# kuwt/edge_alignment

Hardware: AMD Instinct MI355X
Metric: edge-point residual+Jacobian evals/sec (higher is better)
Workload: dtype f64; 1 GPU; c2: single 640x480 frame pair, 50000 edge points, fp64, CauchyLoss(1); points_per_gpu=50000, dt_image=640x480, parallelism=independent frame pairs, one per GPU; single RCCL pose all-gather, tiles=196, points_per_thread=1, lds_bytes=0, point_order_tile_px=0

## Files before the change

### edge_alignment_amd/build.py

```python
import os
import shutil
import subprocess

_HERE = os.path.dirname(os.path.abspath(__file__))
SOURCES = [("csrc/ea_kernels.hip", ["-mllvm", "-amdgpu-sched-strategy=max-ilp"]), ("csrc/ea_kernels_var.hip", []),
           ("csrc/ea_preprocess.hip", []), ("csrc/ea_capi.hip", []), ("csrc/ea_frames.hip", []), ("csrc/ea_comm.hip", [])]
HEADERS = ["csrc/ea_types.h", "csrc/ea_lm.h", "csrc/ea_cov.h", "csrc/ea_prior.h", "csrc/ea_spin.h", "csrc/ea_hip_dev.h",
           "csrc/ea_launch.h", "csrc/ea_poses_map.h", "csrc/ea_wave_exchange.h", "csrc/ea_pair_log.h", "csrc/ea_starts_map.h", "csrc/ea_search_rank.h", "csrc/ea_select.h", "csrc/ea_frame_ws.h", "csrc/ea_capi_internal.h", "../include/ea_hip.h"]
LIB = os.path.join(_HERE, "lib", "libea_hip.so")
FLAGS = ["--offload-arch=gfx950", "-O3", "-std=c++17", "-fno-slp-vectorize", "-fPIC", "-mllvm", "-amdgpu-kernarg-preload-count=16",
         "-Wall", "-Wno-unused-function"]


def _hipcc():
    for cand in (os.environ.get("HIPCC"), "/opt/rocm/bin/hipcc", shutil.which("hipcc")):
        if cand and os.path.exists(cand):
            return cand
    raise RuntimeError("hipcc not found")


def build_library(force=False, verbose=False, out=None, defines=()):
    lib = out or LIB
    srcs = [os.path.join(_HERE, s) for s, _ in SOURCES]
    deps = srcs + [os.path.join(_HERE, h) for h in HEADERS]
    if (not force and os.path.exists(lib)
            and all(os.path.getmtime(lib) >= os.path.getmtime(d) for d in deps)):
        return lib
    obj_dir = os.path.join(os.path.dirname(lib), "obj" + ("_" + os.path.basename(lib) if out else ""))
    os.makedirs(obj_dir, exist_ok=True)
    cc = _hipcc()
    procs, objs = [], []
    for (src, extra), path in zip(SOURCES, srcs):
        obj = os.path.join(obj_dir, os.path.basename(src) + ".o")
        cmd = [cc] + FLAGS + list(extra) + ["-D" + d for d in defines] + ["-c", "-o", obj, path]
        if verbose:
            print(" ".join(cmd))
        procs.append((cmd, subprocess.Popen(cmd, cwd=_HERE)))
        objs.append(obj)
    for cmd, pr in procs:
        if pr.wait() != 0:
            raise subprocess.CalledProcessError(pr.returncode, cmd)
    link = [cc, "--offload-arch=gfx950", "-fPIC", "-shared", "-o", lib] + objs + ["-ldl"]
    if verbose:
        print(" ".join(link))
    subprocess.check_call(link, cwd=_HERE)
    return lib


if __name__ == "__main__":
    print(build_library(force=True, verbose=True))
```

### edge_alignment_amd/csrc/ea_kernels.hip

```cpp

#include <hip/hip_runtime.h>

#include <cstddef>
#include <type_traits>

#if defined(EA_STAMPS) && defined(__HIP_DEVICE_COMPILE__)
namespace ea {
extern __device__ unsigned long long *g_lm_stamp_buf;
extern __device__ int g_lm_probe_row;
}
#define EA_LM_PROBE(k)                                                                              \
  do {                                                                                              \
    if (g_lm_stamp_buf && blockIdx.x == 0) {                                                        \
      unsigned long long t_;                                                                        \
      __builtin_amdgcn_sched_barrier(0);                                                            \
      asm volatile("s_memtime %0\n\ts_waitcnt lgkmcnt(0)" : "=s"(t_)::"memory");                    \
      __builtin_amdgcn_sched_barrier(0);                                                            \
      g_lm_stamp_buf[64 * 8 + g_lm_probe_row * 8 + (k)] = t_;                                       \
    }                                                                                               \
  } while (0)
#endif
#include "ea_launch.h"
#include "ea_poses_map.h"
#include "ea_starts_map.h"
#include "ea_lm.h"
#include "ea_pair_log.h"
#include "ea_prior.h"
#include "ea_select.h"
#include "ea_types.h"
#include "ea_wave_exchange.h"

namespace ea {

#ifdef EA_STAMPS
__device__ unsigned long long *g_stamp_buf = nullptr;
#ifndef EA_STAMPS_EVAL
#define EA_STAMP(slot) do {} while (0)
#else
#define EA_STAMP(slot)                                                                              \
  do {                                                                                              \
    if (g_stamp_buf && threadIdx.x == 0) {                                                          \
      unsigned long long t_;                                                                        \
      __builtin_amdgcn_sched_barrier(0);                                                            \
      asm volatile("s_memtime %0\n\ts_waitcnt lgkmcnt(0)" : "=s"(t_)::"memory");                    \
      __builtin_amdgcn_sched_barrier(0);                                                            \
      g_stamp_buf[((size_t)blockIdx.y * gridDim.x + blockIdx.x) * 8 + (slot)] = t_;                 \
    }                                                                                               \
  } while (0)
#endif
__device__ unsigned long long *g_lm_stamp_buf = nullptr;
__device__ int g_lm_probe_row = 0;
#define EA_LM_STAMP(slot, eval)                                                                     \
  do {                                                                                              \
    if (g_lm_stamp_buf && threadIdx.x == 0 && blockIdx.x == 0) {                                    \
      unsigned long long t_;                                                                        \
      __builtin_amdgcn_sched_barrier(0);                                                            \
      asm volatile("s_memtime %0\n\ts_waitcnt lgkmcnt(0)" : "=s"(t_)::"memory");                    \
      __builtin_amdgcn_sched_barrier(0);                                                            \
      g_lm_stamp_buf[((eval) & 63) * 8 + (slot)] = t_;                                              \
    }                                                                                               \
  } while (0)
#define EA_LM_CLOCK(var)                                                                            \
  unsigned long long var = 0;                                                                       \
  do {                                                                                              \
    __builtin_amdgcn_sched_barrier(0);                                                              \
    asm volatile("s_memtime %0\n\ts_waitcnt lgkmcnt(0)" : "=s"(var)::"memory");                    \
    __builtin_amdgcn_sched_barrier(0);                                                              \
  } while (0)
#define EA_LM_STAMP_PUT(slot, eval, var)                                                            \
  do {                                                                                              \
    if (g_lm_stamp_buf && threadIdx.x == 0 && blockIdx.x == 0) g_lm_stamp_buf[((eval) & 63) * 8 + (slot)] = var; \
  } while (0)
#else
#define EA_STAMP(slot) do {} while (0)
#define EA_LM_STAMP(slot, eval) do {} while (0)
#define EA_LM_CLOCK(var) do {} while (0)
#define EA_LM_STAMP_PUT(slot, eval, var) do {} while (0)
#endif


template <typename T> __device__ __forceinline__ T t_rcp(T x);
template <> __device__ __forceinline__ float t_rcp<float>(float x) { return __builtin_amdgcn_rcpf(x); }
template <> __device__ __forceinline__ double t_rcp<double>(double x) {
  double r = __builtin_amdgcn_rcp(x);
  double e = __builtin_fma(-x, r, 1.0);
  r = __builtin_fma(r, e, r);
  e = __builtin_fma(-x, r, 1.0);
  return __builtin_fma(r, e, r);
}

template <typename T> __device__ __forceinline__ T t_log(T x);
template <> __device__ __forceinline__ float t_log<float>(float x) { return __builtin_amdgcn_logf(x) * 0.6931471805599453f; }

__device__ __forceinline__ double s_const(double c) { asm("" : "+s"(c)); return c; }
__device__ __forceinline__ float s_const(float c) { return c; }

struct LogOps {
  static __device__ __forceinline__ double frexp_mant(double x) { return __builtin_amdgcn_frexp_mant(x); }
  static __device__ __forceinline__ int frexp_exp(double x) { return __builtin_amdgcn_frexp_exp(x); }
  static __device__ __forceinline__ double ldexp(double x, int e) { return __builtin_amdgcn_ldexp(x, e); }
  static __device__ __forceinline__ double rcp(double x) { return __builtin_amdgcn_rcp(x); }
  static __device__ __forceinline__ double sconst(double c) { return s_const(c); }
};
template <> __device__ __forceinline__ double t_log<double>(double x) { return pl_log<LogOps>(x); }

template <typename T> __device__ __forceinline__ T t_sqrt(T x);
template <> __device__ __forceinline__ float t_sqrt<float>(float x) { return __builtin_amdgcn_sqrtf(x); }
template <> __device__ __forceinline__ double t_sqrt<double>(double x) { return sqrt(x); }

template <typename T> __device__ __forceinline__ T t_fma(T a, T b, T c) { return __builtin_fma(a, b, c); }
template <> __device__ __forceinline__ float t_fma<float>(float a, float b, float c) { return __builtin_fmaf(a, b, c); }

template <typename T>
__device__ __forceinline__ void cr_weights(T x, T w[4], T d[4]) {
  const T x2 = x * x;
  const T c15 = s_const(T(1.5));
  w[0] = x * t_fma<T>(x, t_fma<T>(T(-0.5), x, T(1)), T(-0.5));
  w[1] = t_fma<T>(x2, t_fma<T>(c15, x, T(-2.5)), T(1));
  w[2] = x * t_fma<T>(x, t_fma<T>(-c15, x, T(2)), T(0.5));
  w[3] = x2 * t_fma<T>(T(0.5), x, T(-0.5));
  const T c45 = s_const(T(4.5));
  d[0] = t_fma<T>(x, t_fma<T>(-c15, x, T(2)), T(-0.5));
  d[1] = x * t_fma<T>(c45, x, T(-5));
  d[2] = t_fma<T>(x, t_fma<T>(-c45, x, T(4)), T(0.5));
  d[3] = x * t_fma<T>(c15, x, T(-1));
}

template <typename T> struct Uni;
template <> struct Uni<double> {
  static __device__ __forceinline__ const double *R(const PoseState &ps) { return ps.R; }
  static __device__ __forceinline__ const double *t(const PoseState &ps) { return ps.t; }
  static __device__ __forceinline__ const double *G(const PoseState &ps) { return ps.G; }
  static __device__ __forceinline__ double fx(const ProblemDesc &pd) { return pd.fx; }
  static __device__ __forceinline__ double fy(const ProblemDesc &pd) { return pd.fy; }
  static __device__ __forceinline__ double cx(const ProblemDesc &pd) { return pd.cx; }
  static __device__ __forceinline__ double cy(const ProblemDesc &pd) { return pd.cy; }
  static __device__ __forceinline__ double loss_a(const ProblemDesc &pd) { return pd.loss_a; }
  static __device__ __forceinline__ double loss_inv_b(const ProblemDesc &pd) { return pd.loss_inv_b; }
  static __device__ __forceinline__ double z_guard(const ProblemDesc &pd) { return pd.z_guard; }
  static __device__ __forceinline__ double z_eps(const ProblemDesc &pd) { return pd.z_eps; }
  static __device__ __forceinline__ const double *dist(const ProblemDesc &pd) { return pd.dist; }
  static __device__ __forceinline__ const double *A(const ProblemDesc &pd) { return pd.A; }
  static __device__ __forceinline__ const double *d(const ProblemDesc &pd) { return pd.d; }
  static __device__ __forceinline__ const double *Ai(const ProblemDesc &pd) { return pd.Ai; }
  static __device__ __forceinline__ const double *di(const ProblemDesc &pd) { return pd.di; }
};
template <> struct Uni<float> {
  static __device__ __forceinline__ const float *R(const PoseState &ps) { return ps.Rf; }
  static __device__ __forceinline__ const float *t(const PoseState &ps) { return ps.tf; }
  static __device__ __forceinline__ const float *G(const PoseState &ps) { return ps.Gf; }
  static __device__ __forceinline__ float fx(const ProblemDesc &pd) { return pd.fxf; }
  static __device__ __forceinline__ float fy(const ProblemDesc &pd) { return pd.fyf; }
  static __device__ __forceinline__ float cx(const ProblemDesc &pd) { return pd.cxf; }
  static __device__ __forceinline__ float cy(const ProblemDesc &pd) { return pd.cyf; }
  static __device__ __forceinline__ float loss_a(const ProblemDesc &pd) { return pd.loss_af; }
  static __device__ __forceinline__ float loss_inv_b(const ProblemDesc &pd) { return pd.loss_inv_bf; }
  static __device__ __forceinline__ float z_guard(const ProblemDesc &pd) { return pd.z_guardf; }
  static __device__ __forceinline__ float z_eps(const ProblemDesc &pd) { return pd.z_epsf; }
  static __device__ __forceinline__ const float *dist(const ProblemDesc &pd) { return pd.distf; }
  static __device__ __forceinline__ const float *A(const ProblemDesc &pd) { return pd.Af; }
  static __device__ __forceinline__ const float *d(const ProblemDesc &pd) { return pd.df; }
  static __device__ __forceinline__ const float *Ai(const ProblemDesc &pd) { return pd.Aif; }
  static __device__ __forceinline__ const float *di(const ProblemDesc &pd) { return pd.dif; }
};

template <typename T>
struct PoseLite {
  T R[9], t[3];
  int unit_q;
  const PoseState *full;
};
template <typename T> struct PoseAcc {
  static __device__ __forceinline__ const T *R(const PoseState &ps) { return Uni<T>::R(ps); }
  static __device__ __forceinline__ const T *t(const PoseState &ps) { return Uni<T>::t(ps); }
// ... 1236 lines not shown
        v[u] = *reinterpret_cast<const D2 *>(partials + (size_t)min(base + j + u * G, last) * kAccSlots + 2 * id);
    };
    auto add_round = [&](int base, const D2(&v)[U]) {
#pragma unroll
      for (int u = 0; u < U; ++u) {
        const bool in = base + j + u * G <= last;
        s[u].x += in ? v[u].x : 0.0;
        s[u].y += in ? v[u].y : 0.0;
      }
    };
    D2 v0[U], v1[U];
    load_round(tile_begin, v0);
    if (tile_begin + U * G <= last) {
      load_round(tile_begin + U * G, v1);
      add_round(tile_begin, v0);
      add_round(tile_begin + U * G, v1);
      for (int base = tile_begin + 2 * U * G; base <= last; base += U * G) {
        load_round(base, v0);
        add_round(base, v0);
      }
    } else {
      add_round(tile_begin, v0);
    }
  }
#pragma unroll
  for (int w = 1; w < U; w *= 2)
#pragma unroll
    for (int u = 0; u + w < U; u += 2 * w) s[u] += s[u + w];
  *reinterpret_cast<D2 *>(s_part + j * kAccSlots + 2 * id) = s[0];
  __syncthreads();
  if constexpr (F == 1) {
    if (tid < kAccSlots) {
      double tot = 0.0;
#pragma unroll
      for (int k = 0; k < G; ++k) tot += s_part[k * kAccSlots + tid];
      out[tid] = tot;
    }
  } else {
    double *s_fin = s_part + G * kAccSlots;
    if (tid < kAccSlots * F) {
      const int slot = tid & 31, f = tid >> 5;
      double tot = 0.0;
#pragma unroll
      for (int k = 0; k < 16; ++k) tot += s_part[(16 * f + k) * kAccSlots + slot];
      s_fin[f * kAccSlots + slot] = tot;
    }
    __syncthreads();
    if (tid < kAccSlots) {
      double tot = 0.0;
#pragma unroll
      for (int f = 0; f < F; ++f) tot += s_fin[f * kAccSlots + tid];
      out[tid] = tot;
    }
  }
}

__global__ __launch_bounds__(kFoldThreads) void ea_reduce_kernel(const GroupDesc *__restrict__ groups,
                                                                  const double *__restrict__ partials,
                                                                  EvalOut *__restrict__ out) {
  __shared__ __align__(16) double s_part[reduce_tiles_lds<kFoldThreads>()];
  const GroupDesc gd = groups[blockIdx.x];
  reduce_tiles<kFoldThreads, 4>(partials, gd.tile_begin, gd.tile_end, s_part, out[blockIdx.x].acc);
}

__device__ __forceinline__ void signal_done(unsigned int *counter, unsigned int n, int *host_flag, int seq) {
  __threadfence_system();
  const unsigned int prev = __hip_atomic_fetch_add(counter, 1u, __ATOMIC_ACQ_REL, __HIP_MEMORY_SCOPE_AGENT);
  if (prev == n - 1u) {
    __hip_atomic_store(counter, 0u, __ATOMIC_RELAXED, __HIP_MEMORY_SCOPE_AGENT);
    __threadfence_system();
    __hip_atomic_store(host_flag, seq, __ATOMIC_RELEASE, __HIP_MEMORY_SCOPE_SYSTEM);
  }
}

__global__ __launch_bounds__(kFoldThreads) void ea_reduce_done_kernel(const GroupDesc *__restrict__ groups,
                                                                       const double *__restrict__ partials,
                                                                       EvalOut *__restrict__ out, unsigned int *__restrict__ counter,
                                                                       int *__restrict__ host_flag, int seq) {
  __shared__ __align__(16) double s_part[reduce_tiles_lds<kFoldThreads>()];
  const GroupDesc gd = groups[blockIdx.x];
  reduce_tiles<kFoldThreads, 4>(partials, gd.tile_begin, gd.tile_end, s_part, out[blockIdx.x].acc);
  if (threadIdx.x == 0) signal_done(counter, gridDim.x, host_flag, seq);
}

__global__ __launch_bounds__(kLmThreads) void ea_reduce256_kernel(const GroupDesc *__restrict__ groups,
                                                                  const double *__restrict__ partials,
                                                                  EvalOut *__restrict__ out) {
  __shared__ __align__(16) double s_part[reduce_tiles_lds<kLmThreads>()];
  const GroupDesc gd = groups[blockIdx.x];
  reduce_tiles<kLmThreads, 4>(partials, gd.tile_begin, gd.tile_end, s_part, out[blockIdx.x].acc);
}

template <typename T, int PPT, int NT, bool BUF, bool IMG32 = false>
__global__ __launch_bounds__(NT) void ea_eval_fold_kernel(
    const void *__restrict__ x0, const void *__restrict__ y0, const void *__restrict__ z0, int n0,
    int shape, int chunks_per_xcd,
    const ProblemDesc *__restrict__ probs, const PoseState *__restrict__ poses,
    double *__restrict__ partials, int lds_texels,
    const GroupDesc *__restrict__ groups, const double *__restrict__ prev_rows, EvalOut *__restrict__ prev_out) {
  if (blockIdx.x == gridDim.x - 1) {
    __shared__ __align__(16) double s_part[reduce_tiles_lds<NT>()];
    const GroupDesc gd = groups[blockIdx.y];
    reduce_tiles<NT, 4>(prev_rows, gd.tile_begin, gd.tile_end, s_part, prev_out[blockIdx.y].acc);
    return;
  }
  eval_fused_body<T, PPT, 0, NT, false, BUF, IMG32>(x0, y0, z0, n0, shape, chunks_per_xcd, probs, poses, partials, lds_texels);
}

template <int NT>
__device__ __forceinline__ void poses_fold_one(const PosesFold &f, int r) {
  __shared__ __align__(16) double s_part[reduce_tiles_lds<NT>()];
  int pose, problem;
  poses_rider(r, f.count, &pose, &problem);
  const GroupDesc gd = f.groups[problem];
  const int base = pose * f.rows_per_pose;
  reduce_tiles<NT, 4>(f.rows, base + gd.tile_begin, base + gd.tile_end, s_part, f.out[r].acc);
  if (threadIdx.x == 0) signal_done(f.counter, (unsigned)f.n, f.host_flag, f.seq);
}

template <typename T, int PPT, int MODE, int NT, bool VAR, bool BUF, bool IMG32 = false>
__global__ __launch_bounds__(NT) void ea_eval_poses_kernel(
    const void *__restrict__ x0, const void *__restrict__ y0, const void *__restrict__ z0, int n0,
    int shape, int g, int rows,
    const ProblemDesc *__restrict__ probs, const PoseState *__restrict__ poses,
    double *__restrict__ partials, PosesFold fold) {
  static_assert((MODE == 0 || MODE == kModeExchange) && !VAR, "plain functor, stencil rows from L2");
  constexpr bool XCHG = MODE == kModeExchange;
  extern __shared__ __align__(16) unsigned char smem[];
  double *s_red = reinterpret_cast<double *>(smem);
  int *s_box = reinterpret_cast<int *>(smem + kRedBytes);
  const PosesWork w = poses_work(blockIdx.x, shape, rows, g, fold.n);
  if (w.kind != 2) {
    if (w.kind == 1) poses_fold_one<NT>(fold, w.rider);
    return;
  }
  const PosesChunk pc = poses_chunk(w, shape, rows, reinterpret_cast<const PosesRow *>(probs) - rows);
  const int tid = threadIdx.x;
  EA_ITEM_HEAD(false, NT * PPT, pc.chunk, pc.term, pc.slot, false, return);
  const double sum = fused_chunk<T, PPT, 0, NT, false, BUF, IMG32, PoseLite<T>, XCHG>(pd, ps, X, Y, Z, count, s_red, s_box, (T *)nullptr, 0,
                                                                                       tid < kAccSlots ? tid : -1);
  store_row_sum<XCHG>(partials, pc.out_row, sum);
}

template <int NT>
__global__ __launch_bounds__(NT) void ea_poses_fold_kernel(PosesFold fold) {
  poses_fold_one<NT>(fold, blockIdx.x);
}

template <typename T> using CPtr = const T __attribute__((address_space(4))) *;
constexpr int kLanesWaves = 4, kLanesSub = 512 / kLanesWaves, kLanesVals = 29;

template <typename IT> struct LanesStage {
  double cx_, cy_, cz_, iz, fu, fv;
  bool valid;
  Row4<IT> row[4];
};
template <typename IT> __device__ __forceinline__ Row4<double> lanes_widen(const Row4<IT> &r) {
  Row4<double> o;
  o.p0 = (double)r.p0; o.p1 = (double)r.p1; o.p2 = (double)r.p2; o.p3 = (double)r.p3;
  return o;
}
template <bool BUF, bool IMG32>
__device__ __forceinline__ void lanes_stage(const ProblemDesc &pd, const PoseLite<double> &ps, double x, double y, double z,
                                            bool inb, LanesStage<typename ImgOf<double, IMG32>::type> &st, int &n_bad) {
  typedef double T;
  typedef typename ImgOf<T, IMG32>::type IT;
  const int pitch = pd.pitch;
  const void *img_base = IMG32 ? pd.dt32 : pd.dt;
  Proj<T> pr;
  project_point<T>(pd, ps, x, y, z, pr);
  st.valid = inb && pr.state == 1;
  n_bad += (inb && pr.state == 2) ? 1 : 0;
  if (__any(!st.valid)) {
    asm volatile("" ::: "memory");
    if (!st.valid) { pr.iu = 0; pr.iv = 0; pr.fu = T(0); pr.fv = T(0); }
  }
  st.cx_ = pr.cx_; st.cy_ = pr.cy_; st.cz_ = pr.cz_; st.iz = pr.iz; st.fu = pr.fu; st.fv = pr.fv;
  if constexpr (BUF) {
    const __amdgpu_buffer_rsrc_t rimg =
        make_raw_buffer(img_base, (unsigned)pitch * (unsigned)(pd.H + 2 * kImagePad) * (unsigned)sizeof(IT));
    const int voff = ((pr.iv + (kImagePad - 1)) * pitch + (pr.iu + (kImagePad - 1))) * (int)sizeof(IT);
#pragma unroll
    for (int l = 0; l < 4; ++l) st.row[l] = buf_load_row4<IT>(rimg, voff, l * pitch * (int)sizeof(IT));
  } else {
    const GPtr<IT> gimg = (GPtr<IT>)(static_cast<const IT *>(img_base) + (size_t)kImagePad * (size_t)pitch + kImagePad);
    const GPtr<IT> base = gimg + ((ptrdiff_t)(pr.iv - 1) * pitch + (pr.iu - 1));
#pragma unroll
    for (int l = 0; l < 4; ++l) st.row[l] = load_row4<IT>(base + (ptrdiff_t)l * pitch);
  }
}
struct LanesLogRun { double P, L; int E; };
template <bool IMG32, bool UNIT>
__device__ __forceinline__ void lanes_sums(int k, const ProblemDesc &pd, const PoseLite<double> &ps_, double x, double y, double z,
                                           const LanesStage<typename ImgOf<double, IMG32>::type> &st, bool pair,
                                           double (&acc)[28], double &cost, double &held, LanesLogRun &run,
                                           const double (*s_pose)[64]) {
  typedef double T;
  PoseLite<T> ps = ps_;
  if constexpr (UNIT) ps.unit_q = 1;
  const T loss_a = Uni<T>::loss_a(pd);
  Proj<T> pr;
  pr.cx_ = st.cx_; pr.cy_ = st.cy_; pr.cz_ = st.cz_; pr.iz = st.iz; pr.fu = st.fu; pr.fv = st.fv;
  if constexpr (UNIT) {
    asm volatile("" ::: "memory");
    ps.t[0] = s_pose[10][threadIdx.x & 63]; ps.t[1] = s_pose[11][threadIdx.x & 63];
  }
  pr.bx = st.cx_ + ps.t[0]; pr.by = st.cy_ + ps.t[1];
  pr.fxz = Uni<T>::fx(pd) * st.iz; pr.fyz = Uni<T>::fy(pd) * st.iz;
  if (__any(!st.valid)) {
    asm volatile("" ::: "memory");
    if (!st.valid) {
      pr.iz = T(1);
      pr.bx = T(0); pr.by = T(0);
      pr.fxz = T(0); pr.fyz = T(0);
    }
  }
  T f, Fu, Fv;
  bicubic<T>(pr.fu, pr.fv, [&](int l) { return lanes_widen(st.row[l]); }, f, Fu, Fv);
  T J[6];
  jacobian_row<T>(pd, ps, pr, x, y, z, Fu, Fv, J);
  T rho, w;
  if (UNIT && pair) {
    const T xs = (f * f) * Uni<T>::loss_inv_b(pd);
    rho = xs + T(1);
    w = t_rcp<T>(rho);
    if (__any(!st.valid)) {
      asm volatile("" ::: "memory");
      if (!st.valid) { w = T(0); rho = T(1); }
    }
    T p = run.P * rho;
    const bool high = pl_run_high<LogOps>(p);
    if (__any(high)) {
      asm volatile("" ::: "memory");
      if (high) p = pl_run_renorm<LogOps>(run.P, run.L, run.E, rho);
    }
    pl_run_take(run.P, run.L, rho, p);
  } else {
    loss_point<T, 2, false>(pair, pd.loss_kind, loss_a, Uni<T>::loss_inv_b(pd), f * f, st.valid, T(1), rho, w);
  }
  const T wr = w * f;
  int s = 0;
#pragma unroll
  for (int a = 0; a < 6; ++a) {
    const T wJa = w * J[a];
#pragma unroll
    for (int b = a; b < 6; ++b) { acc[s] = t_fma<T>(wJa, J[b], acc[s]); ++s; }
    acc[kAccJtr + a] = t_fma<T>(J[a], wr, acc[kAccJtr + a]);
  }
  if (!(UNIT && pair)) cost_point<T, 2>(k, pair, loss_a, rho, cost, held);
}

template <bool BUF, bool IMG32, bool UNIT>
__device__ __forceinline__ void lanes_run(const ProblemDesc &pd, const PoseLite<double> &ps_, CPtr<double> px, CPtr<double> py,
                                          CPtr<double> pz, int n_sub, bool pair, double (&acc)[28], int &n_bad,
                                          const double (*s_pose)[64]) {
  typedef double T;
  typedef typename ImgOf<T, IMG32>::type IT;
  if (n_sub <= 0) return;
  const int lane = threadIdx.x & 63;
  n_sub = __builtin_amdgcn_readfirstlane(n_sub);
  const int last = n_sub - 1;
  LanesLogRun run = {T(1), T(0), 0};
  T X[2], Y[2], Z[2], NX[2], NY[2], NZ[2];
  {
    const int i1 = min(1, last), i2 = min(2, last), i3 = min(3, last);
    X[0] = px[0]; X[1] = px[i1]; Y[0] = py[0]; Y[1] = py[i1]; Z[0] = pz[0]; Z[1] = pz[i1];
    NX[0] = px[i2]; NX[1] = px[i3]; NY[0] = py[i2]; NY[1] = py[i3]; NZ[0] = pz[i2]; NZ[1] = pz[i3];
  }
#pragma nounroll
  for (int i = 0; i < n_sub; i += 2) {
    const int i4 = min(i + 4, last), i5 = min(i + 5, last);
    const T FX[2] = {px[i4], px[i5]}, FY[2] = {py[i4], py[i5]}, FZ[2] = {pz[i4], pz[i5]};
    T held = T(1), cost = T(0);
    LanesStage<IT> A, B;
    PoseLite<T> ps = ps_;
    if constexpr (UNIT) {
      asm volatile("" ::: "memory");
#pragma unroll
      for (int k = 0; k < 9; ++k) ps.R[k] = s_pose[k][lane];
      ps.t[2] = s_pose[9][lane]; ps.t[0] = s_pose[10][lane]; ps.t[1] = s_pose[11][lane];
    }
    lanes_stage<BUF, IMG32>(pd, ps, X[0], Y[0], Z[0], true, A, n_bad);
    if constexpr (UNIT) lanes_stage<BUF, IMG32>(pd, ps, X[1], Y[1], Z[1], i + 1 < n_sub, B, n_bad);
    lanes_sums<IMG32, UNIT>(0, pd, ps, X[0], Y[0], Z[0], A, pair, acc, cost, held, run, s_pose);
    if constexpr (!UNIT) lanes_stage<BUF, IMG32>(pd, ps, X[1], Y[1], Z[1], i + 1 < n_sub, B, n_bad);
    lanes_sums<IMG32, UNIT>(1, pd, ps, X[1], Y[1], Z[1], B, pair, acc, cost, held, run, s_pose);
    if (!(UNIT && pair)) acc[kAccCost] += cost;
#pragma unroll
    for (int k = 0; k < 2; ++k) { X[k] = NX[k]; Y[k] = NY[k]; Z[k] = NZ[k]; NX[k] = FX[k]; NY[k] = FY[k]; NZ[k] = FZ[k]; }
  }
  if (UNIT && pair) acc[kAccCost] = (T(0.5) * (Uni<T>::loss_a(pd) * Uni<T>::loss_a(pd))) * pl_run_log<LogOps>(run.P, run.L, run.E);
}

__device__ __forceinline__ bool lanes_ticket(unsigned int *counter, unsigned int target, volatile int *s_word) {
  asm volatile("s_waitcnt vmcnt(0)" ::: "memory");
  __syncthreads();
  if (threadIdx.x == 0) {
    __builtin_amdgcn_fence(__ATOMIC_RELEASE, "agent");
    asm volatile("s_waitcnt vmcnt(0)" ::: "memory");
    const unsigned int prev = __hip_atomic_fetch_add(counter, 1u, __ATOMIC_RELAXED, __HIP_MEMORY_SCOPE_AGENT);
    const int last = prev + 1u == target;
    if (last) {
      __builtin_amdgcn_fence(__ATOMIC_ACQUIRE, "agent");
      asm volatile("s_waitcnt vmcnt(0)" ::: "memory");
    }
    *s_word = last;
  }
  __syncthreads();
  return *s_word != 0;
}
constexpr int kLanesFoldSlots = (kLanesVals + kLanesWaves - 1) / kLanesWaves;
__device__ __forceinline__ void lanes_fold_blocks(const double *src, size_t stride, int n, int wave, int lane, double (&v)[kLanesFoldSlots]) {
#pragma unroll
  for (int j = 0; j < kLanesFoldSlots; ++j) v[j] = 0.0;
  const double *p = src + lane;
  int r = 0;
  for (; r + 4 <= n; r += 4) {
    double x[4][kLanesFoldSlots];
#pragma unroll
    for (int u = 0; u < 4; ++u)
#pragma unroll
      for (int j = 0; j < kLanesFoldSlots; ++j) {
        const int slot = wave + kLanesWaves * j;
        x[u][j] = slot < kLanesVals ? p[(size_t)(r + u) * stride + (size_t)slot * kPosesLanes] : 0.0;
      }
#pragma unroll
    for (int u = 0; u < 4; ++u)
#pragma unroll
      for (int j = 0; j < kLanesFoldSlots; ++j) v[j] += x[u][j];
  }
  for (; r < n; ++r) {
    double x[kLanesFoldSlots];
#pragma unroll
    for (int j = 0; j < kLanesFoldSlots; ++j) {
      const int slot = wave + kLanesWaves * j;
      x[j] = slot < kLanesVals ? p[(size_t)r * stride + (size_t)slot * kPosesLanes] : 0.0;
    }
#pragma unroll
    for (int j = 0; j < kLanesFoldSlots; ++j) v[j] += x[j];
  }
}
__device__ __forceinline__ void lanes_tickets(const PosesTickets &tk, const double *rows_base, int rows, int group, int problem,
                                              int row0, int nrows, int chunk, int pose0, int live, int groups, double *s_lds) {
  const int lane = threadIdx.x & 63, wave = __builtin_amdgcn_readfirstlane(threadIdx.x >> 6);
  volatile int *s_word = reinterpret_cast<volatile int *>(s_lds);
  const int count = tk.count, run = poses_lanes_run(chunk), slot1 = poses_lanes_run_slot(row0, problem, run);
  if (!lanes_ticket(tk.counters + poses_lanes_counter1(group, slot1, rows, count), (unsigned)poses_lanes_run_rows(nrows, run), s_word)) return;
  double v[kLanesFoldSlots];
  lanes_fold_blocks(rows_base + poses_lanes_row_off(group, row0 + run * kPosesRun, rows), (size_t)kPosesLanesBlock,
                    poses_lanes_run_rows(nrows, run), wave, lane, v);
  double *part = tk.partials + poses_lanes_partial_off(group, slot1, rows, count);
#pragma unroll
  for (int j = 0; j < kLanesFoldSlots; ++j) {
    const int slot = wave + kLanesWaves * j;
    if (slot < kLanesVals) part[(size_t)slot * kPosesLanes + lane] = v[j];
  }
  if (!lanes_ticket(tk.counters + poses_lanes_counter2(groups, group, problem, rows, count), (unsigned)poses_lanes_runs(nrows), s_word)) return;
  lanes_fold_blocks(tk.partials + poses_lanes_partial_off(group, poses_lanes_run_slot(row0, problem, 0), rows, count),
                    (size_t)kPosesLanesBlock, poses_lanes_runs(nrows), wave, lane, v);
  __syncthreads();
  static_assert(kLanesFoldSlots * kLanesWaves == kAccSlots, "the wavefronts' slots cover a result exactly");
#pragma unroll
  for (int j = 0; j < kLanesFoldSlots; ++j) {
    const int slot = wave + kLanesWaves * j;
    s_lds[slot * 65 + lane] = slot < kLanesVals ? v[j] : 0.0;
  }
  __syncthreads();
  {
    const int s = threadIdx.x & (kAccSlots - 1), p0 = threadIdx.x / kAccSlots;
#pragma unroll
    for (int it = 0; it < kPosesLanes / (64 * kLanesWaves / kAccSlots); ++it) {
      const int p = p0 + it * (64 * kLanesWaves / kAccSlots);
      if (p < live) tk.out[(size_t)(pose0 + p) * (size_t)count + (size_t)problem].acc[s] = s_lds[s * 65 + p];
    }
  }
  __threadfence_system();
  __syncthreads();
  if (threadIdx.x == 0) {
    __threadfence_system();
    __hip_atomic_store(tk.flags + poses_lanes_flag(tk.group0 + group, problem, count), tk.seq, __ATOMIC_RELEASE, __HIP_MEMORY_SCOPE_SYSTEM);
  }
}

template <bool BUF, bool IMG32>
__global__ __launch_bounds__(64 * kLanesWaves) __attribute__((amdgpu_waves_per_eu(2, 2))) void ea_eval_poses_lanes_kernel(
    int shape, int g, int rows, const ProblemDesc *__restrict__ probs, const PoseState *__restrict__ poses,
    double *rows_out, PosesTickets tk) {
  typedef double T;
  __shared__ __align__(16) double s_sum[kLanesWaves / 2][kLanesVals][64];
  __shared__ __align__(16) double s_pose[kLanesWaves][12][64];
  static_assert(sizeof(s_sum) >= sizeof(double) * kAccSlots * 65, "the fold's transposition fits the sums' array");
  const PosesLanesWork w = poses_lanes_work(blockIdx.x, shape, rows, g, 0);
  if (w.kind != 2) return;
  const PosesLanesChunk pc = poses_lanes_chunk(w.row, shape, reinterpret_cast<const PosesRow *>(probs) - rows);
  const ProblemDesc pd = probs[pc.term];
  const long long start = (long long)pc.chunk * (kLanesWaves * kLanesSub);
  const int count = (int)max(0ll, min((long long)(kLanesWaves * kLanesSub), (long long)pd.n - start));
  const int lane = threadIdx.x & 63, wave = __builtin_amdgcn_readfirstlane(threadIdx.x >> 6);
  const PoseState *psp = poses + ((size_t)(w.pose0 + min(lane, w.live - 1)) * (size_t)pc.count + (size_t)pc.term);
  PoseLite<T> ps;
  int active;
  load_pose_lite<T>(psp, ps, active);
  const bool on = lane < w.live && active != 0;

  T v[kLanesVals];
#pragma unroll
  for (int i = 0; i < kLanesVals; ++i) v[i] = T(0);
  if (__any(on)) {
    const int first = wave * kLanesSub, n_sub = max(0, min(kLanesSub, count - first));
    const CPtr<T> px = (CPtr<T>)(static_cast<const T *>(pd.x) + start + first);
    const CPtr<T> py = (CPtr<T>)(static_cast<const T *>(pd.y) + start + first);
    const CPtr<T> pz = (CPtr<T>)(static_cast<const T *>(pd.z) + start + first);
    const bool pair = pd.loss_kind == 1;
    T acc[28];
#pragma unroll
    for (int i = 0; i < 28; ++i) acc[i] = T(0);
    int n_bad = 0;
#pragma unroll
    for (int k = 0; k < 9; ++k) s_pose[wave][k][lane] = ps.R[k];
    s_pose[wave][9][lane] = ps.t[2]; s_pose[wave][10][lane] = ps.t[0]; s_pose[wave][11][lane] = ps.t[1];
    if (__all(ps.unit_q != 0)) lanes_run<BUF, IMG32, true>(pd, ps, px, py, pz, n_sub, pair, acc, n_bad, s_pose[wave]);
    else lanes_run<BUF, IMG32, false>(pd, ps, px, py, pz, n_sub, pair, acc, n_bad, s_pose[wave]);

#pragma unroll
    for (int i = 0; i < 28; ++i) v[i] = acc[i];
    v[28] = (T)n_bad;
#pragma unroll
    for (int s = 1; s < kLanesWaves; s <<= 1) {
      const int role = wave & (2 * s - 1), buf = wave / (2 * s);
      if (role == s) {
#pragma unroll
        for (int i = 0; i < kLanesVals; ++i) s_sum[buf][i][lane] = v[i];
      }
      __syncthreads();
      if (role == 0) {
#pragma unroll
        for (int i = 0; i < kLanesVals; ++i) v[i] += s_sum[buf][i][lane];
      }
      if (2 * s < kLanesWaves) __syncthreads();
    }
  }
  const int group = w.pose0 / kPosesLanes;
  if (wave == 0) {
    double *o = rows_out + poses_lanes_row_off(group, w.row, rows) + lane;
#pragma unroll
    for (int i = 0; i < kLanesVals; ++i) o[(size_t)i * kPosesLanes] = on ? v[i] : 0.0;
  }
  if (!tk.on) return;
  lanes_tickets(tk, rows_out, rows, group, pc.term, w.row - pc.chunk, pd.tile_end - pd.tile_begin, pc.chunk, w.pose0, w.live,
                poses_lanes_groups(g), &s_sum[0][0][0]);
}


template <typename T>
__device__ __forceinline__ void cr_weights_value(T x, T w[4]) {
  const T x2 = x * x;
  const T c15 = s_const(T(1.5));
  w[0] = x * t_fma<T>(x, t_fma<T>(T(-0.5), x, T(1)), T(-0.5));
  w[1] = t_fma<T>(x2, t_fma<T>(c15, x, T(-2.5)), T(1));
  w[2] = x * t_fma<T>(x, t_fma<T>(-c15, x, T(2)), T(0.5));
  w[3] = x2 * t_fma<T>(T(0.5), x, T(-0.5));
}
template <typename T, typename RowFn>
__device__ __forceinline__ T bicubic_value(T fu, T fv, RowFn row) {
  T wu[4], wv[4];
  cr_weights_value<T>(fu, wu);
  cr_weights_value<T>(fv, wv);
  T f = T(0);
#pragma unroll
  for (int l = 0; l < 4; ++l) {
    const Row4<T> r = row(l);
    const T rs = t_fma<T>(wu[3], r.p3, t_fma<T>(wu[2], r.p2, t_fma<T>(wu[1], r.p1, wu[0] * r.p0)));
    f = t_fma<T>(wv[l], rs, f);
  }
  return f;
}

template <int CTRL> __device__ __forceinline__ int lane_xchg(int x) { return __builtin_amdgcn_update_dpp(0, x, CTRL, 0xF, 0xF, true); }
template <int W>
__device__ __forceinline__ void swap_rows_b32(unsigned &a, unsigned &b) {
  if constexpr (W == 32) asm volatile("s_nop 1\n\tv_permlane32_swap_b32 %0, %1\n\ts_nop 0" : "+v"(a), "+v"(b));
  else asm volatile("s_nop 1\n\tv_permlane16_swap_b32 %0, %1\n\ts_nop 0" : "+v"(a), "+v"(b));
}
template <int W> __device__ __forceinline__ float swap_add(float x) {
  unsigned a = __builtin_bit_cast(unsigned, x), b = a;
  swap_rows_b32<W>(a, b);
  return __builtin_bit_cast(float, a) + __builtin_bit_cast(float, b);
}
template <int W> __device__ __forceinline__ int swap_add(int x) {
  unsigned a = (unsigned)x, b = a;
  swap_rows_b32<W>(a, b);
  return (int)(a + b);
}
template <int W> __device__ __forceinline__ double swap_add(double x) {
  const unsigned long long u = __builtin_bit_cast(unsigned long long, x);
  unsigned al = (unsigned)u, ah = (unsigned)(u >> 32), bl = al, bh = ah;
  if constexpr (W == 32)
    asm volatile("s_nop 1\n\tv_permlane32_swap_b32 %0, %2\n\tv_permlane32_swap_b32 %1, %3\n\ts_nop 0" : "+v"(al), "+v"(ah), "+v"(bl), "+v"(bh));
  else
    asm volatile("s_nop 1\n\tv_permlane16_swap_b32 %0, %2\n\tv_permlane16_swap_b32 %1, %3\n\ts_nop 0" : "+v"(al), "+v"(ah), "+v"(bl), "+v"(bh));
  return __builtin_bit_cast(double, ((unsigned long long)ah << 32) | al) + __builtin_bit_cast(double, ((unsigned long long)bh << 32) | bl);
}
template <typename V>
__device__ __forceinline__ V wave_sum1(V x) {
  x += lane_xchg<kDppQuadXor1>(x);
  x += lane_xchg<kDppQuadXor2>(x);
  x += lane_xchg<kDppRowHalfMirror>(x);
  x += lane_xchg<kDppRowMirror>(x);
  x = swap_add<16>(x);
  return swap_add<32>(x);
}
template <int NT, typename A, typename B>
__device__ __forceinline__ void workgroup_sum2(A a, B b, double &total_a, B &total_b) {
  __shared__ double s_a[NT / 64];
  __shared__ B s_b[NT / 64];
  const int tid = threadIdx.x;
  const A wa = wave_sum1<A>(a);
  const B wb = wave_sum1<B>(b);
  if ((tid & 63) == 0) { s_a[tid >> 6] = (double)wa; s_b[tid >> 6] = wb; }
  __syncthreads();
  if (tid == 0) {
    double ta = 0.0;
    B tb = 0;
#pragma unroll
    for (int v = 0; v < NT / 64; ++v) { ta += s_a[v]; tb += s_b[v]; }
    total_a = ta; total_b = tb;
  }
}

struct __attribute__((aligned(16))) CostPartial { double cost, failed; };
static_assert(sizeof(CostPartial) == kCostPartialBytes, "ea_launch.h");

template <typename T, int PPT, int NT, bool BUF, bool IMG32>
__device__ __forceinline__ bool cost_item(const void *__restrict__ x0, const void *__restrict__ y0, const void *__restrict__ z0, int n0,
                                          const ProblemDesc *__restrict__ probs, const PoseState *__restrict__ poses,
                                          const PosesChunk &pc, CostPartial *__restrict__ partials) {
  typedef typename ImgOf<T, IMG32>::type IT;
  const int tid = threadIdx.x;
  EA_ITEM_HEAD(false, NT * PPT, pc.chunk, pc.term, pc.slot, false, return false);
  const int pitch = pd.pitch;
  const void *img_base = IMG32 ? pd.dt32 : pd.dt;
  const GPtr<IT> gimg = (GPtr<IT>)(static_cast<const IT *>(img_base) + (size_t)kImagePad * (size_t)pitch + kImagePad);
  const __amdgpu_buffer_rsrc_t rimg =
      make_raw_buffer(img_base, BUF ? (unsigned)pitch * (unsigned)(pd.H + 2 * kImagePad) * (unsigned)sizeof(IT) : 0u);
  const int loss_kind = pd.loss_kind;
  const T loss_a = Uni<T>::loss_a(pd), loss_inv_b = Uni<T>::loss_inv_b(pd);
  Proj<T> pr[PPT];
  bool valid[PPT];
  int n_bad = 0;
#pragma unroll
  for (int k = 0; k < PPT; ++k) {
    const bool inb = tid + k * NT < count;
    project_point<T>(pd, ps, X[k], Y[k], Z[k], pr[k]);
    valid[k] = inb && pr[k].state == 1;
    n_bad += (inb && pr[k].state == 2) ? 1 : 0;
    if (__any(!valid[k]) && !valid[k]) {
      pr[k].iu = 0; pr[k].iv = 0; pr[k].fu = T(0); pr[k].fv = T(0);
    }
  }
  T acc = T(0), held = T(1);
  const bool pair = loss_kind == 1;
#pragma unroll
  for (int k = 0; k < PPT; ++k) {
    T f;
    if constexpr (BUF) {
      const int voff = ((pr[k].iv + (kImagePad - 1)) * pitch + (pr[k].iu + (kImagePad - 1))) * (int)sizeof(IT);
      f = bicubic_value<T>(pr[k].fu, pr[k].fv, [&](int l) { return RowLoad<T, IT>::buf(rimg, voff, l * pitch * (int)sizeof(IT)); });
    } else {
      const GPtr<IT> base = gimg + ((ptrdiff_t)(pr[k].iv - 1) * pitch + (pr[k].iu - 1));
      f = bicubic_value<T>(pr[k].fu, pr[k].fv, [&](int l) { return RowLoad<T, IT>::flat(base + (ptrdiff_t)l * pitch); });
    }
    T rho, wt;
    loss_point<T, PPT, false>(pair, loss_kind, loss_a, loss_inv_b, f * f, valid[k], T(1), rho, wt);
    cost_point<T, PPT>(k, pair, loss_a, rho, acc, held);
  }
// ... 1126 lines not shown
```

Baseline: 105.2 billion evals/s.

## Restructure lanes point loop: ballot masks, shallower prefetch, drop LDS pose reloads

Rewrites the per-wave point streaming loop in the poses-lanes kernel. Validity becomes a scalar ballot mask instead of a per-lane bool. Point coordinates are prefetched one pair ahead instead of two, using paired 16-byte loads when aligned. The pose matrix is no longer spilled to and reloaded from LDS each iteration, and the next coordinate load is placed inside the second point's sums. The aim is lower VGPR pressure and fewer LDS and VMEM instructions per point, at the cost of a shorter latency-hiding distance for the coordinate loads.

```diff
diff --git a/edge_alignment_amd/build.py b/edge_alignment_amd/build.py
--- a/edge_alignment_amd/build.py
+++ b/edge_alignment_amd/build.py
@@ -6,7 +6,7 @@
 SOURCES = [("csrc/ea_kernels.hip", ["-mllvm", "-amdgpu-sched-strategy=max-ilp"]), ("csrc/ea_kernels_var.hip", []),
            ("csrc/ea_preprocess.hip", []), ("csrc/ea_capi.hip", []), ("csrc/ea_frames.hip", []), ("csrc/ea_comm.hip", [])]
 HEADERS = ["csrc/ea_types.h", "csrc/ea_lm.h", "csrc/ea_cov.h", "csrc/ea_prior.h", "csrc/ea_spin.h", "csrc/ea_hip_dev.h",
-           "csrc/ea_launch.h", "csrc/ea_poses_map.h", "csrc/ea_wave_exchange.h", "csrc/ea_pair_log.h", "csrc/ea_starts_map.h", "csrc/ea_search_rank.h", "csrc/ea_select.h", "csrc/ea_frame_ws.h", "csrc/ea_capi_internal.h", "../include/ea_hip.h"]
+           "csrc/ea_launch.h", "csrc/ea_poses_map.h", "csrc/ea_lanes_stream.h", "csrc/ea_wave_exchange.h", "csrc/ea_pair_log.h", "csrc/ea_starts_map.h", "csrc/ea_search_rank.h", "csrc/ea_select.h", "csrc/ea_frame_ws.h", "csrc/ea_capi_internal.h", "../include/ea_hip.h"]
 LIB = os.path.join(_HERE, "lib", "libea_hip.so")
 FLAGS = ["--offload-arch=gfx950", "-O3", "-std=c++17", "-fno-slp-vectorize", "-fPIC", "-mllvm", "-amdgpu-kernarg-preload-count=16",
          "-Wall", "-Wno-unused-function"]
diff --git a/edge_alignment_amd/csrc/ea_kernels.hip b/edge_alignment_amd/csrc/ea_kernels.hip
--- a/edge_alignment_amd/csrc/ea_kernels.hip
+++ b/edge_alignment_amd/csrc/ea_kernels.hip
@@ -20,6 +20,7 @@
     }                                                                                               \
   } while (0)
 #endif
+#include "ea_lanes_stream.h"
 #include "ea_launch.h"
 #include "ea_poses_map.h"
 #include "ea_starts_map.h"
@@ -1562,9 +1563,14 @@
 
 template <typename IT> struct LanesStage {
   double cx_, cy_, cz_, iz, fu, fv;
-  bool valid;
+  unsigned long long bad;
   Row4<IT> row[4];
 };
+__device__ __forceinline__ bool lanes_any(unsigned long long &m) {
+  asm volatile("" : "+s"(m));
+  return m != 0;
+}
+__device__ __forceinline__ bool lanes_mine(unsigned long long m) { return __builtin_amdgcn_inverse_ballot_w64(m); }
 template <typename IT> __device__ __forceinline__ Row4<double> lanes_widen(const Row4<IT> &r) {
   Row4<double> o;
   o.p0 = (double)r.p0; o.p1 = (double)r.p1; o.p2 = (double)r.p2; o.p3 = (double)r.p3;
@@ -1579,11 +1585,12 @@
   const void *img_base = IMG32 ? pd.dt32 : pd.dt;
   Proj<T> pr;
   project_point<T>(pd, ps, x, y, z, pr);
-  st.valid = inb && pr.state == 1;
+  const bool valid = inb && pr.state == 1;
   n_bad += (inb && pr.state == 2) ? 1 : 0;
-  if (__any(!st.valid)) {
+  st.bad = __builtin_amdgcn_ballot_w64(!valid);
+  if (lanes_any(st.bad)) {
     asm volatile("" ::: "memory");
-    if (!st.valid) { pr.iu = 0; pr.iv = 0; pr.fu = T(0); pr.fv = T(0); }
+    if (lanes_mine(st.bad)) { pr.iu = 0; pr.iv = 0; pr.fu = T(0); pr.fv = T(0); }
   }
   st.cx_ = pr.cx_; st.cy_ = pr.cy_; st.cz_ = pr.cz_; st.iz = pr.iz; st.fu = pr.fu; st.fv = pr.fv;
   if constexpr (BUF) {
@@ -1600,43 +1607,41 @@
   }
 }
 struct LanesLogRun { double P, L; int E; };
-template <bool IMG32, bool UNIT>
+template <bool IMG32, bool UNIT, typename Under>
 __device__ __forceinline__ void lanes_sums(int k, const ProblemDesc &pd, const PoseLite<double> &ps_, double x, double y, double z,
                                            const LanesStage<typename ImgOf<double, IMG32>::type> &st, bool pair,
-                                           double (&acc)[28], double &cost, double &held, LanesLogRun &run,
-                                           const double (*s_pose)[64]) {
+                                           double (&acc)[28], double &cost, double &held, LanesLogRun &run, Under under) {
   typedef double T;
   PoseLite<T> ps = ps_;
   if constexpr (UNIT) ps.unit_q = 1;
   const T loss_a = Uni<T>::loss_a(pd);
+  unsigned long long bad = st.bad;
   Proj<T> pr;
   pr.cx_ = st.cx_; pr.cy_ = st.cy_; pr.cz_ = st.cz_; pr.iz = st.iz; pr.fu = st.fu; pr.fv = st.fv;
-  if constexpr (UNIT) {
-    asm volatile("" ::: "memory");
-    ps.t[0] = s_pose[10][threadIdx.x & 63]; ps.t[1] = s_pose[11][threadIdx.x & 63];
-  }
   pr.bx = st.cx_ + ps.t[0]; pr.by = st.cy_ + ps.t[1];
   pr.fxz = Uni<T>::fx(pd) * st.iz; pr.fyz = Uni<T>::fy(pd) * st.iz;
-  if (__any(!st.valid)) {
+  if (lanes_any(bad)) {
     asm volatile("" ::: "memory");
-    if (!st.valid) {
+    if (lanes_mine(bad)) {
       pr.iz = T(1);
       pr.bx = T(0); pr.by = T(0);
       pr.fxz = T(0); pr.fyz = T(0);
     }
   }
+  under();
   T f, Fu, Fv;
   bicubic<T>(pr.fu, pr.fv, [&](int l) { return lanes_widen(st.row[l]); }, f, Fu, Fv);
   T J[6];
   jacobian_row<T>(pd, ps, pr, x, y, z, Fu, Fv, J);
+  if constexpr (UNIT) asm volatile("" ::"v"(J[0]), "v"(J[1]), "v"(J[2]), "v"(J[3]), "v"(J[4]), "v"(J[5]));
   T rho, w;
   if (UNIT && pair) {
     const T xs = (f * f) * Uni<T>::loss_inv_b(pd);
     rho = xs + T(1);
     w = t_rcp<T>(rho);
-    if (__any(!st.valid)) {
+    if (lanes_any(bad)) {
       asm volatile("" ::: "memory");
-      if (!st.valid) { w = T(0); rho = T(1); }
+      if (lanes_mine(bad)) { w = T(0); rho = T(1); }
     }
     T p = run.P * rho;
     const bool high = pl_run_high<LogOps>(p);
@@ -1646,7 +1651,9 @@
     }
     pl_run_take(run.P, run.L, rho, p);
   } else {
-    loss_point<T, 2, false>(pair, pd.loss_kind, loss_a, Uni<T>::loss_inv_b(pd), f * f, st.valid, T(1), rho, w);
+    if constexpr (UNIT) asm volatile("" ::: "memory");
+    loss_point<T, 2, false>(pair, pd.loss_kind, loss_a, Uni<T>::loss_inv_b(pd), f * f, !lanes_mine(bad), T(1), rho, w);
+    cost_point<T, 2>(k, pair, loss_a, rho, cost, held);
   }
   const T wr = w * f;
   int s = 0;
@@ -1657,47 +1664,52 @@
     for (int b = a; b < 6; ++b) { acc[s] = t_fma<T>(wJa, J[b], acc[s]); ++s; }
     acc[kAccJtr + a] = t_fma<T>(J[a], wr, acc[kAccJtr + a]);
   }
-  if (!(UNIT && pair)) cost_point<T, 2>(k, pair, loss_a, rho, cost, held);
 }
 
 template <bool BUF, bool IMG32, bool UNIT>
-__device__ __forceinline__ void lanes_run(const ProblemDesc &pd, const PoseLite<double> &ps_, CPtr<double> px, CPtr<double> py,
-                                          CPtr<double> pz, int n_sub, bool pair, double (&acc)[28], int &n_bad,
-                                          const double (*s_pose)[64]) {
+__device__ __forceinline__ void lanes_run(const ProblemDesc &pd, const PoseLite<double> &ps, CPtr<double> px, CPtr<double> py,
+                                          CPtr<double> pz, int n_sub, bool pair, double (&acc)[28], int &n_bad) {
   typedef double T;
   typedef typename ImgOf<T, IMG32>::type IT;
+  typedef T T2 __attribute__((ext_vector_type(2), aligned(8)));
   if (n_sub <= 0) return;
-  const int lane = threadIdx.x & 63;
   n_sub = __builtin_amdgcn_readfirstlane(n_sub);
-  const int last = n_sub - 1;
+  const int iters = lanes_stream_iters(n_sub);
   LanesLogRun run = {T(1), T(0), 0};
-  T X[2], Y[2], Z[2], NX[2], NY[2], NZ[2];
-  {
-    const int i1 = min(1, last), i2 = min(2, last), i3 = min(3, last);
-    X[0] = px[0]; X[1] = px[i1]; Y[0] = py[0]; Y[1] = py[i1]; Z[0] = pz[0]; Z[1] = pz[i1];
-    NX[0] = px[i2]; NX[1] = px[i3]; NY[0] = py[i2]; NY[1] = py[i3]; NZ[0] = pz[i2]; NZ[1] = pz[i3];
-  }
+  const auto load_pair = [&](int k, T (&x)[2], T (&y)[2], T (&z)[2]) {
+    const LanesStreamLoad ld = lanes_stream_load(k, n_sub);
+    if (ld.wide) {
+      const T2 vx = *(const CPtr<T2>)(px + ld.i0), vy = *(const CPtr<T2>)(py + ld.i0), vz = *(const CPtr<T2>)(pz + ld.i0);
+      x[0] = vx.x; x[1] = vx.y; y[0] = vy.x; y[1] = vy.y; z[0] = vz.x; z[1] = vz.y;
+    } else {
+      asm volatile("" ::: "memory");
+      x[0] = px[ld.i0]; x[1] = px[ld.i1]; y[0] = py[ld.i0]; y[1] = py[ld.i1]; z[0] = pz[ld.i0]; z[1] = pz[ld.i1];
+    }
+  };
+  T X[2], Y[2], Z[2];
+  load_pair(-1, X, Y, Z);
 #pragma nounroll
-  for (int i = 0; i < n_sub; i += 2) {
-    const int i4 = min(i + 4, last), i5 = min(i + 5, last);
-    const T FX[2] = {px[i4], px[i5]}, FY[2] = {py[i4], py[i5]}, FZ[2] = {pz[i4], pz[i5]};
-    T held = T(1), cost = T(0);
+  for (int k = 0; k < iters; ++k) {
+    T held, cost;
     LanesStage<IT> A, B;
-    PoseLite<T> ps = ps_;
+    lanes_stage<BUF, IMG32>(pd, ps, X[0], Y[0], Z[0], true, A, n_bad);
     if constexpr (UNIT) {
+      lanes_stage<BUF, IMG32>(pd, ps, X[1], Y[1], Z[1], 2 * k + 1 < n_sub, B, n_bad);
+      lanes_sums<IMG32, true>(0, pd, ps, T(0), T(0), T(0), A, pair, acc, cost, held, run, []() {});
+      lanes_sums<IMG32, true>(1, pd, ps, T(0), T(0), T(0), B, pair, acc, cost, held, run, [&]() { load_pair(k, X, Y, Z); });
+    } else {
+      T NX[2], NY[2], NZ[2];
+      load_pair(k, NX, NY, NZ);
+      lanes_sums<IMG32, false>(0, pd, ps, X[0], Y[0], Z[0], A, pair, acc, cost, held, run, []() {});
+      lanes_stage<BUF, IMG32>(pd, ps, X[1], Y[1], Z[1], 2 * k + 1 < n_sub, B, n_bad);
+      lanes_sums<IMG32, false>(1, pd, ps, X[1], Y[1], Z[1], B, pair, acc, cost, held, run, []() {});
+#pragma unroll
+      for (int j = 0; j < 2; ++j) { X[j] = NX[j]; Y[j] = NY[j]; Z[j] = NZ[j]; }
+    }
+    if (!(UNIT && pair)) {
       asm volatile("" ::: "memory");
-#pragma unroll
-      for (int k = 0; k < 9; ++k) ps.R[k] = s_pose[k][lane];
-      ps.t[2] = s_pose[9][lane]; ps.t[0] = s_pose[10][lane]; ps.t[1] = s_pose[11][lane];
-    }
-    lanes_stage<BUF, IMG32>(pd, ps, X[0], Y[0], Z[0], true, A, n_bad);
-    if constexpr (UNIT) lanes_stage<BUF, IMG32>(pd, ps, X[1], Y[1], Z[1], i + 1 < n_sub, B, n_bad);
-    lanes_sums<IMG32, UNIT>(0, pd, ps, X[0], Y[0], Z[0], A, pair, acc, cost, held, run, s_pose);
-    if constexpr (!UNIT) lanes_stage<BUF, IMG32>(pd, ps, X[1], Y[1], Z[1], i + 1 < n_sub, B, n_bad);
-    lanes_sums<IMG32, UNIT>(1, pd, ps, X[1], Y[1], Z[1], B, pair, acc, cost, held, run, s_pose);
-    if (!(UNIT && pair)) acc[kAccCost] += cost;
-#pragma unroll
-    for (int k = 0; k < 2; ++k) { X[k] = NX[k]; Y[k] = NY[k]; Z[k] = NZ[k]; NX[k] = FX[k]; NY[k] = FY[k]; NZ[k] = FZ[k]; }
+      acc[kAccCost] += cost;
+    }
   }
   if (UNIT && pair) acc[kAccCost] = (T(0.5) * (Uni<T>::loss_a(pd) * Uni<T>::loss_a(pd))) * pl_run_log<LogOps>(run.P, run.L, run.E);
 }
@@ -1798,7 +1810,6 @@
     double *rows_out, PosesTickets tk) {
   typedef double T;
   __shared__ __align__(16) double s_sum[kLanesWaves / 2][kLanesVals][64];
-  __shared__ __align__(16) double s_pose[kLanesWaves][12][64];
   static_assert(sizeof(s_sum) >= sizeof(double) * kAccSlots * 65, "the fold's transposition fits the sums' array");
   const PosesLanesWork w = poses_lanes_work(blockIdx.x, shape, rows, g, 0);
   if (w.kind != 2) return;
@@ -1826,11 +1837,8 @@
 #pragma unroll
     for (int i = 0; i < 28; ++i) acc[i] = T(0);
     int n_bad = 0;
-#pragma unroll
-    for (int k = 0; k < 9; ++k) s_pose[wave][k][lane] = ps.R[k];
-    s_pose[wave][9][lane] = ps.t[2]; s_pose[wave][10][lane] = ps.t[0]; s_pose[wave][11][lane] = ps.t[1];
-    if (__all(ps.unit_q != 0)) lanes_run<BUF, IMG32, true>(pd, ps, px, py, pz, n_sub, pair, acc, n_bad, s_pose[wave]);
-    else lanes_run<BUF, IMG32, false>(pd, ps, px, py, pz, n_sub, pair, acc, n_bad, s_pose[wave]);
+    if (__all(ps.unit_q != 0)) lanes_run<BUF, IMG32, true>(pd, ps, px, py, pz, n_sub, pair, acc, n_bad);
+    else lanes_run<BUF, IMG32, false>(pd, ps, px, py, pz, n_sub, pair, acc, n_bad);
 
 #pragma unroll
     for (int i = 0; i < 28; ++i) v[i] = acc[i];
diff --git a/edge_alignment_amd/csrc/ea_lanes_stream.h b/edge_alignment_amd/csrc/ea_lanes_stream.h
--- /dev/null
+++ b/edge_alignment_amd/csrc/ea_lanes_stream.h
@@ -0,0 +1,18 @@
+#pragma once
+#include "ea_types.h"
+
+namespace ea {
+
+struct LanesStreamLoad {
+  int i0, i1;
+  int wide;
+};
+EA_HD inline int lanes_stream_iters(int n_sub) { return (n_sub + 1) >> 1; }
+EA_HD inline LanesStreamLoad lanes_stream_pair(int k, int n_sub) {
+  const int last = n_sub - 1, i = 2 * k;
+  if (i + 1 <= last) return LanesStreamLoad{i, i + 1, 1};
+  return LanesStreamLoad{last, last, 0};
+}
+EA_HD inline LanesStreamLoad lanes_stream_load(int k, int n_sub) { return lanes_stream_pair(k + 1, n_sub); }
+
+}
```

New measurement: 115.7 billion evals/s, median of 6. 1.1x the previous value.
